# mataiyuan/ASD-SLAM

Measured on AMD Instinct MI355X. Metric: frames/sec end-to-end tracking+LocalBA, KITTI 00 mono @2000 keypoints, higher is better.
Workload: dtype f32

## Files before the change

### asd-slam_amd/csrc/asdnet.hip

```cpp
#include "ctx.h"

#include <algorithm>
#include <cmath>
#include <cstring>

typedef float f32x16 __attribute__((ext_vector_type(16)));
typedef float f32x4 __attribute__((ext_vector_type(4)));


namespace {

struct LayerSpec { int cout, cin, k, stride, pad; };
const LayerSpec kLayers[7] = {{32, 1, 3, 1, 1},   {32, 32, 3, 1, 1},   {64, 32, 3, 2, 1},  {64, 64, 3, 1, 1},
                              {128, 64, 3, 2, 1}, {128, 128, 3, 1, 1}, {128, 128, 8, 1, 0}};

template <int CIN, int COUT, int HIN, int S, int ROWS, int WM, int WN, int KC, int PP = 1, int RING = 2>
struct ConvCfg {
  static constexpr int HO = HIN / S;
  static constexpr int INROWS = (ROWS - 1) * S + 3;
  static constexpr int INCOLS = (HO - 1) * S + 3;
  static constexpr int CPAD = CIN + 4;
  static constexpr int NW = WM * WN;
  static constexpr int NTH = 64 * NW;
  static constexpr int M_PATCH = ROWS * HO;
// ... 412 lines not shown


constexpr float kActScale = 16.f;

typedef _Float16 f16x8 __attribute__((ext_vector_type(8)));
__device__ inline void split8_f16(const f32x4& v0, const f32x4& v1, float scale, u32x4& ph, u32x4& pl) {
  float x[8] = {v0[0], v0[1], v0[2], v0[3], v1[0], v1[1], v1[2], v1[3]};
  f16x8 h, l;
#pragma unroll
  for (int j = 0; j < 8; ++j) {
    const float xs = x[j] * scale;
    h[j] = (_Float16)xs;
    l[j] = (_Float16)(xs - (float)h[j]);
  }
  ph = __builtin_bit_cast(u32x4, h);
  pl = __builtin_bit_cast(u32x4, l);
}

__device__ __forceinline__ void split4_mix(float x0, float x1, float x2, float x3, float s, uint32_t (&h)[2], uint32_t (&l)[2]) {
  asm("v_fma_mixlo_f16 %0, %8, %4, 0\n\t"
      "v_fma_mixlo_f16 %1, %8, %6, 0\n\t"
      "v_fma_mixhi_f16 %0, %8, %5, 0\n\t"
      "v_fma_mixhi_f16 %1, %8, %7, 0\n\t"
      "v_fma_mixlo_f16 %2, %8, %4, -%0 op_sel_hi:[0,0,1]\n\t"
      "v_fma_mixlo_f16 %3, %8, %6, -%1 op_sel_hi:[0,0,1]\n\t"
      "v_fma_mixhi_f16 %2, %8, %5, -%0 op_sel:[0,0,1] op_sel_hi:[0,0,1]\n\t"
      "v_fma_mixhi_f16 %3, %8, %7, -%1 op_sel:[0,0,1] op_sel_hi:[0,0,1]\n\t"
      "s_nop 0"
      : "=&v"(h[0]), "=&v"(h[1]), "=&v"(l[0]), "=&v"(l[1])
      : "v"(x0), "v"(x1), "v"(x2), "v"(x3), "s"(s));
}


__global__ __launch_bounds__(256) void k_patch_stats(const uint8_t* __restrict__ patches, float* __restrict__ stats, int n) {
  __shared__ float red[8];
  const int t = threadIdx.x, lane = t & 63, wave = t >> 6, patch = blockIdx.x;
  const uchar4 v = reinterpret_cast<const uchar4*>(patches + (size_t)patch * 1024)[t];
  const float inv255 = (float)(1.0 / 255);
  float x[4] = {v.x * inv255, v.y * inv255, v.z * inv255, v.w * inv255};
#pragma unroll
  for (int k = 0; k < 4; ++k) asm volatile("" : "+v"(x[k]));
  float sum = (x[0] + x[1]) + (x[2] + x[3]);
  for (int off = 32; off >= 1; off >>= 1) sum += __shfl_xor(sum, off);
  if (lane == 0) red[wave] = sum;
  asd_syncthreads();
  const float mean = ((red[0] + red[1]) + (red[2] + red[3])) * (1.0f / 1024.0f);
  float d[4], ss = 0.f;
  for (int k = 0; k < 4; ++k) { d[k] = x[k] - mean; ss += d[k] * d[k]; }
  for (int off = 32; off >= 1; off >>= 1) ss += __shfl_xor(ss, off);
  if (lane == 0) red[4 + wave] = ss;
  asd_syncthreads();
  const float sd = sqrtf(((red[4] + red[5]) + (red[6] + red[7])) * (1.0f / 1023.0f)) + 1e-7f;
  if (t == 0) { stats[2 * (size_t)patch] = mean; stats[2 * (size_t)patch + 1] = sd; }
}

template <int CIN, int COUT, int HIN, int S, int ROWS, int WM, int WN, int PP, bool FUSE1 = false, int NP = 3, bool PAIR = false>
__device__ __forceinline__ void conv_x3_tile(const int bid, const void* __restrict__ in_, const uint8_t* __restrict__ wimg,
                                                         const float* __restrict__ bias, float* __restrict__ out,
                                                         const float* __restrict__ w1, const float* __restrict__ b1, int n,
                                                         unsigned long long* __restrict__ stamps, float in_scale, float out_scale,
                                                         const float* __restrict__ stats = nullptr) {
  using C = X3Cfg<CIN, COUT, HIN, S, ROWS, WM, WN, PP, NP>;
  constexpr int NTH = C::NTH, MT = C::MT, NCW = C::NCW;
  static_assert(!PAIR || NP == 2, "the pair format belongs to the two-piece form");
  extern __shared__ __attribute__((aligned(16))) uint8_t smem_b[];
  int t = threadIdx.x;
  asm volatile("" : "+v"(t));
  const int lane = t & 63, wave = t >> 6;
  const int wm = wave / WN, wn = wave % WN;
  constexpr int BANDS = C::HO / ROWS;
  const int patch = (bid / BANDS) * PP, band = bid % BANDS;
  const int r0 = band * ROWS;
  unsigned long long st_t0 = 0, st_t1 = 0;
  if (stamps) st_t0 = st_t1 = __builtin_amdgcn_s_memtime();
#define X3_STAMP(k) do { if (stamps && t == 0) stamps[16 * bid + (k)] = __builtin_amdgcn_s_memtime() - st_t0; } while (0)

  constexpr int SUB = 2, KG = C::KCH / 8, TW = 32 / SUB;
  const int kg = lane >> 4, lr = lane & 15;
  const uint8_t* wl = wimg + ((size_t)kg * COUT + wn * NCW + lr) * 16;
  constexpr int NB = NCW / TW;
  auto load_b = [&](int c, u32x4 (&b)[NB][NP]) {
    const uint8_t* wc = wl + (size_t)c * C::CHUNKB;
#pragma unroll
    for (int nb = 0; nb < NB; ++nb)
#pragma unroll
      for (int p = 0; p < NP; ++p) b[nb][p] = *reinterpret_cast<const u32x4*>(wc + (size_t)p * KG * COUT * 16 + nb * TW * 16);
  };
  constexpr int RB = C::NCHUNK % ASD_X3_RB == 0 ? ASD_X3_RB : 3;
  static_assert(C::NCHUNK % RB == 0, "chunk count");
  u32x4 br[RB][NB][NP];
#pragma unroll
  for (int d = 0; d < RB - 1; ++d) load_b(d, br[d]);

  if constexpr (FUSE1) {
    static_assert(!FUSE1 || (CIN == 32 && HIN == 32 && S == 1 && PP == 1 && (C::NW == 4 || C::NW == 8)), "conv1 fusion is for conv2 only");
    float* pin = reinterpret_cast<float*>(smem_b + C::ACT_BYTES);
    float* wsh = pin + (ROWS + 4) * 36;
    float* red = wsh + 320;
    const uint8_t* patches = static_cast<const uint8_t*>(in_);
    for (int i = t; i < (ROWS + 4) * 36; i += NTH) {
      const int j = i / 36, c = i % 36, y = r0 - 2 + j;
      if (!(c >= 1 && c <= 32 && y >= 0 && y < 32)) pin[i] = 0.f;
    }
    for (int i = t; i < 288; i += NTH) wsh[i] = w1[i];
    if (t < 32) wsh[288 + t] = b1[t];
    const bool ld = C::NW == 4 || wave < 4;
    const uchar4 v = ld ? reinterpret_cast<const uchar4*>(patches + (size_t)patch * 1024)[t] : make_uchar4(0, 0, 0, 0);
    const float inv255 = (float)(1.0 / 255);
    float x[4] = {v.x * inv255, v.y * inv255, v.z * inv255, v.w * inv255};
#pragma unroll
    for (int k = 0; k < 4; ++k) asm volatile("" : "+v"(x[k]));
    float d[4], sd;
    if (stats) {
      const float mean = stats[2 * (size_t)patch];
      sd = stats[2 * (size_t)patch + 1];
      for (int k = 0; k < 4; ++k) d[k] = x[k] - mean;
      X3_STAMP(9);
    } else {
      float sum = (x[0] + x[1]) + (x[2] + x[3]);
      for (int off = 32; off >= 1; off >>= 1) sum += __shfl_xor(sum, off);
      X3_STAMP(9);
      if (lane == 0 && ld) red[wave] = sum;
      asd_syncthreads();
      const float mean = ((red[0] + red[1]) + (red[2] + red[3])) * (1.0f / 1024.0f);
      float ss = 0.f;
      for (int k = 0; k < 4; ++k) { d[k] = x[k] - mean; ss += d[k] * d[k]; }
      for (int off = 32; off >= 1; off >>= 1) ss += __shfl_xor(ss, off);
      if (lane == 0 && ld) red[4 + wave] = ss;
      asd_syncthreads();
      sd = sqrtf(((red[4] + red[5]) + (red[6] + red[7])) * (1.0f / 1023.0f)) + 1e-7f;
    }
    if (ld) {
      const int idx = t * 4, y = idx >> 5, x0 = idx & 31;
      const int j = y - (r0 - 2);
      if (j >= 0 && j < ROWS + 4)
        for (int k = 0; k < 4; ++k) pin[j * 36 + x0 + k + 1] = d[k] / sd;
    }
    asd_syncthreads();
    if (stamps) st_t1 = __builtin_amdgcn_s_memtime();
    constexpr int NPIX = C::INROWS * C::INCOLS;
    const int q = t & 3;
    float wq[8][9], bq1[8];
#pragma unroll
    for (int c = 0; c < 8; ++c) {
      bq1[c] = wsh[288 + 8 * q + c];
#pragma unroll
      for (int k = 0; k < 9; ++k) wq[c][k] = wsh[(8 * q + c) * 9 + k];
    }
    for (int item = t; item < NPIX * 4; item += NTH) {
      const int pix = item >> 2;
      const int i = pix % C::INCOLS, j = pix / C::INCOLS;
      const int oy = r0 - 1 + j, ox = i - 1;
      f32x4 ra = {0.f, 0.f, 0.f, 0.f}, rb = {0.f, 0.f, 0.f, 0.f};
      if (oy >= 0 && oy < 32 && ox >= 0 && ox < 32) {
        float a[9];
#pragma unroll
        for (int ky = 0; ky < 3; ++ky)
#pragma unroll
          for (int kx = 0; kx < 3; ++kx) a[ky * 3 + kx] = pin[(j + ky) * 36 + ox + kx];
#pragma unroll
        for (int c = 0; c < 8; ++c) {
          float acc1 = bq1[c];
#pragma unroll
          for (int k = 0; k < 9; ++k) acc1 += a[k] * wq[c][k];
          const float r = acc1 > 0.f ? acc1 : 0.f;
          if (c < 4) ra[c] = r; else rb[c - 4] = r;
        }
      }
      u32x4 ph, pm, pl;
      uint8_t* dst = smem_b + pix * C::PIXB + q * C::GSTR;
      if constexpr (NP == 2) {
        split8_f16(ra, rb, in_scale, ph, pl);
        *reinterpret_cast<u32x4*>(dst) = ph;
        *reinterpret_cast<u32x4*>(dst + C::PSTR) = pl;
      } else {
        split8(ra, rb, ph, pm, pl);
        *reinterpret_cast<u32x4*>(dst) = ph;
        *reinterpret_cast<u32x4*>(dst + 16) = pm;
        *reinterpret_cast<u32x4*>(dst + 32) = pl;
      }
    }
  } else if constexpr (PAIR) {
    const uint8_t* inb = static_cast<const uint8_t*>(in_) + (size_t)patch * HIN * HIN * CIN * 4;
    constexpr int C8 = CIN / 8;
    constexpr int NPIXB = C::INROWS * C::INCOLS;
    static_assert(NTH % C8 == 0, "a thread keeps its channel group");
    constexpr int PSTEP = NTH / C8;
// ... 135 lines not shown
#pragma unroll
      for (int ma = 0; ma < NA; ++ma) {
        const int q = u * NA + ma;
        const int qn = q + PD;
        load_a(abase[qn % NA] + offs[qn / NA], ar[qn % RS]);
        const u32x4 (&ac)[NP] = ar[q % RS];
#pragma unroll
        for (int nb = 0; nb < NB; ++nb) {
          if constexpr (NP == 2) {
            mma(ac[1], bc[nb][0], acc[ma][nb]);
            mma(ac[0], bc[nb][1], acc[ma][nb]);
            mma(ac[0], bc[nb][0], acc[ma][nb]);
          } else {
            mma(ac[2], bc[nb][0], acc[ma][nb]);
            mma(ac[0], bc[nb][2], acc[ma][nb]);
            mma(ac[1], bc[nb][1], acc[ma][nb]);
            mma(ac[1], bc[nb][0], acc[ma][nb]);
            mma(ac[0], bc[nb][1], acc[ma][nb]);
            mma(ac[0], bc[nb][0], acc[ma][nb]);
          }
        }
#pragma unroll
        for (int p = 0; p < NP; ++p) {
          __builtin_amdgcn_sched_group_barrier(0x008, (NP * (NP + 1) / 2) * NB / NP, 0);
          __builtin_amdgcn_sched_group_barrier(0x100, 1, 0);
        }
      }
    }
  }

  if (stamps) {
    asm volatile("s_nop 0" ::"v"(acc[NA - 1][NB - 1][0]));
    const unsigned long long e_c = __builtin_amdgcn_s_memtime(), e_r = __builtin_amdgcn_s_memrealtime();
    if (t == 0) { stamps[16 * bid] = e_c - st_c; stamps[16 * bid + 1] = e_r - st_r; stamps[16 * bid + 2] = st_t1 - st_t0; stamps[16 * bid + 3] = st_c - st_t1; stamps[16 * bid + 6] = st_t0; }
  }
  if constexpr (PAIR) {
    uint8_t* opb = reinterpret_cast<uint8_t*>(out) + ((size_t)patch * C::HO + r0) * C::HO * COUT * 4;
    for (int nb = 0; nb < NB; ++nb) {
      const int co0 = wn * NCW + nb * TW + 4 * kg;
      const f32x4 bv = *reinterpret_cast<const f32x4*>(bias + co0);
      for (int ma = 0; ma < NA; ++ma) {
        const int m0 = wm * MT * 32 + ma * TW;
        const int pp = PP > 1 ? m0 / C::M_PATCH : 0;
        if (PP > 1 && patch + pp >= n) continue;
        const int m = tile_pixel(m0 / TW, lr);
        float v[4];
#pragma unroll
        for (int r = 0; r < 4; ++r) { const float x = acc[ma][nb][r] * out_scale + bv[r]; v[r] = x < 0.f ? 0.f : x; }
        uint32_t hh[2], ll[2];
        split4_mix(v[0], v[1], v[2], v[3], kActScale, hh, ll);
        const auto s0 = __builtin_amdgcn_permlane16_swap(hh[0], ll[0], false, false);
        const auto s1 = __builtin_amdgcn_permlane16_swap(hh[1], ll[1], false, false);
        uint8_t* o = opb + ((size_t)pp * C::HO * C::HO + (size_t)(m - pp * C::M_PATCH)) * COUT * 4 + (co0 >> 3) * 32 + (kg & 1) * 16;
        *reinterpret_cast<u32x4*>(o) = u32x4{s0[0], s1[0], s0[1], s1[1]};
      }
    }
  } else {
  float* op = out + ((size_t)patch * C::HO + r0) * C::HO * COUT;
  for (int nb = 0; nb < NB; ++nb) {
    const int co = wn * NCW + nb * TW + lr;
    const float bv = bias[co];
    for (int ma = 0; ma < NA; ++ma) {
      const int m0 = wm * MT * 32 + ma * TW;
      const int pp = PP > 1 ? m0 / C::M_PATCH : 0;
      if (PP > 1 && patch + pp >= n) continue;
      for (int r = 0; r < AR; ++r) {
        const int m = tile_pixel(m0 / TW, 4 * kg + r);
        const size_t o = (size_t)pp * C::HO * C::HO * COUT + (size_t)(m - pp * C::M_PATCH) * COUT + co;
        const float v = (NP == 2 ? acc[ma][nb][r] * out_scale : acc[ma][nb][r]) + bv;
        op[o] = NP == 2 ? (v < 0.f ? 0.f : v) : (v > 0.f ? v : 0.f);
      }
    }
  }
  }
  if (stamps && t == 0) { const unsigned long long e = __builtin_amdgcn_s_memtime(); stamps[16 * bid + 5] = e - st_t0; stamps[16 * bid + 7] = e; }
}

#ifndef ASD_L2_MINWG
#define ASD_L2_MINWG 3
#endif
template <int CIN, int COUT, int HIN, int S, int ROWS, int WM, int WN, int PP, bool FUSE1 = false, int NP = 3, bool PAIR = false>
__global__ __launch_bounds__(64 * WM * WN, (FUSE1 && NP == 2) ? ASD_L2_MINWG : 1) void k_conv_x3(const void* __restrict__ in_, const uint8_t* __restrict__ wimg,
                                                         const float* __restrict__ bias, float* __restrict__ out,
                                                         const float* __restrict__ w1, const float* __restrict__ b1, int n,
                                                         unsigned long long* __restrict__ stamps, float in_scale, float out_scale,
                                                         const float* __restrict__ stats) {
  const int bid = (S == 2 && CIN == 32) ? (int)(gridDim.x - 1 - blockIdx.x) : (int)blockIdx.x;
  conv_x3_tile<CIN, COUT, HIN, S, ROWS, WM, WN, PP, FUSE1, NP, PAIR>(bid, in_, wimg, bias, out, w1, b1, n, stamps, in_scale, out_scale, stats);
}

constexpr int FC_SK = 16;
constexpr int FC_KCH = 128;
constexpr int FC_MT = 1;
__global__ __launch_bounds__(256) void k_fc_mfma(const float* __restrict__ act, const float* __restrict__ wimg,
                                                 float* __restrict__ part, int n, int npad) {
  __shared__ __attribute__((aligned(16))) float sa[FC_MT * 32 * (FC_KCH + 4)];
  const int t = threadIdx.x, lane = t & 63, wave = t >> 6;
  const int h = lane >> 5, li = lane & 31;
  const int p0 = blockIdx.x * 32 * FC_MT, sk = blockIdx.y;
  constexpr int KPER = 8192 / FC_SK;
  f32x16 acc[FC_MT];
  for (int m = 0; m < FC_MT; ++m)
    for (int r = 0; r < 16; ++r) acc[m][r] = 0.f;
  for (int st = 0; st < KPER / FC_KCH; ++st) {
    const int k0 = sk * KPER + st * FC_KCH;
    asd_syncthreads();
    for (int idx = t; idx < FC_MT * 32 * (FC_KCH / 4); idx += 256) {
      const int c4 = idx % (FC_KCH / 4), row = idx / (FC_KCH / 4);
      int p = p0 + row;
      if (p >= n) p = n - 1;
      *reinterpret_cast<f32x4*>(sa + row * (FC_KCH + 4) + c4 * 4) =
          *reinterpret_cast<const f32x4*>(act + (size_t)p * 8192 + k0 + c4 * 4);
    }
    asd_syncthreads();
    const float* wb = wimg + ((size_t)(k0 / 8) * 2 + h) * 128 * 4 + (wave * 32 + li) * 4;
#pragma unroll 4
    for (int c8 = 0; c8 < FC_KCH / 8; ++c8) {
      const f32x4 b = *reinterpret_cast<const f32x4*>(wb + (size_t)c8 * 2 * 128 * 4);
      f32x4 a[FC_MT];
#pragma unroll
      for (int m = 0; m < FC_MT; ++m) a[m] = *reinterpret_cast<const f32x4*>(sa + (m * 32 + li) * (FC_KCH + 4) + c8 * 8 + 4 * h);
// ... 199 lines not shown
                                                float* __restrict__ desc, int n, int npad, int* __restrict__ range_flag) {
  const int lane = threadIdx.x & 63, p = blockIdx.x * 4 + (threadIdx.x >> 6);
  if (p >= n) return;
  float v0 = 0.f, v1 = 0.f;
  for (int sk = 0; sk < FC_SK; ++sk) {
    v0 += part[((size_t)sk * npad + p) * 128 + lane];
    v1 += part[((size_t)sk * npad + p) * 128 + lane + 64];
  }
  v0 += bias[lane];
  v1 += bias[lane + 64];
  float ss = v0 * v0 + v1 * v1;
  for (int off = 32; off >= 1; off >>= 1) ss += __shfl_xor(ss, off);
  const float norm = sqrtf(ss + 1e-10f);
  if (range_flag && lane == 0 && !(fabsf(ss) <= 3.0e38f)) *range_flag = 1;
  desc[(size_t)p * 128 + lane] = v0 / norm;
  desc[(size_t)p * 128 + lane + 64] = v1 / norm;
}

#define L2_CFG 32, 32, 32, 1, 4, 4, 1, 16, 1, 3
#define L3_CFG 32, 64, 32, 2, 4, 2, 2, 16
#define L4_CFG 64, 64, 16, 1, 8, 4, 1, 32, 1, 2
#define L5_CFG 64, 128, 16, 2, 4, 1, 4, 16, 1, 3
#define L6_CFG 128, 128, 8, 1, 8, 2, 2, 16, 1, 3
#ifndef ASD_L2_WMN
#define ASD_L2_WMN 4, 1
#endif
#ifndef ASD_L3_WMN
#define ASD_L3_WMN 1, 4
#endif
#ifndef ASD_L4_WMN
#define ASD_L4_WMN 2, 2
#endif
#define L2S_CFG 32, 32, 32, 1, 8, ASD_L2_WMN, 1
#ifndef ASD_L3_ROWS
#define ASD_L3_ROWS 4
#endif
#define L3S_CFG 32, 64, 32, 2, ASD_L3_ROWS, ASD_L3_WMN, 1
#define L4S_CFG 64, 64, 16, 1, 8, ASD_L4_WMN, 1
#ifndef ASD_L5_RWMN
#define ASD_L5_RWMN 8, 1, 4
#endif
#ifndef ASD_L6_WMN
#define ASD_L6_WMN 1, 4
#endif
#define L5S_CFG 64, 128, 16, 2, ASD_L5_RWMN, 1
#define L6S_CFG 128, 128, 8, 1, 8, ASD_L6_WMN, 1

template <int CIN, int COUT, int HIN, int S, int ROWS, int WM, int WN, int KC, int PP = 1, int RING = 2, bool FUSE1 = false>
hipError_t launch_conv(hipStream_t st, const void* in, const float* wimg, const float* bias, float* out, int n,
                       const float* w1 = nullptr, const float* b1 = nullptr) {
  using C = ConvCfg<CIN, COUT, HIN, S, ROWS, WM, WN, KC, PP, RING>;
  auto kern = k_conv_mfma<CIN, COUT, HIN, S, ROWS, WM, WN, KC, PP, RING, FUSE1>;
  constexpr int lds = C::LDS_BYTES + (FUSE1 ? ((ROWS + 4) * 36 + 320 + 8) * 4 : 0);
  static_assert(lds <= 160 * 1024, "band + weight ring do not fit LDS");
  static AsdPerDeviceOnce attr_set;
  int dev_ = 0;
  (void)hipGetDevice(&dev_);
  if (attr_set.need(dev_)) {
    hipError_t e = hipFuncSetAttribute(reinterpret_cast<const void*>(kern), hipFuncAttributeMaxDynamicSharedMemorySize, lds);
    if (e != hipSuccess) return e;
    attr_set.done(dev_);
  }
  hipLaunchKernelGGL(kern, dim3(((n + PP - 1) / PP) * (C::HO / ROWS)), dim3(C::NTH), lds, st, in, wimg, bias, out, w1, b1, n);
  return hipGetLastError();
}

template <int CIN, int COUT, int HIN, int S, int ROWS, int WM, int WN, int KC>
hipError_t launch_conv_p(hipStream_t st, const float* in, const float* wimg, const float* bias, float* out, int n, int num_cu) {
  using C = ConvCfg<CIN, COUT, HIN, S, ROWS, WM, WN, KC>;
  auto kern = k_conv_mfma_p<CIN, COUT, HIN, S, ROWS, WM, WN, KC>;
  constexpr int lds = (2 * C::ACT_FLOATS + 2 * C::WCHUNK) * 4;
  static_assert(lds <= 160 * 1024, "double-buffered band does not fit LDS");
  static AsdPerDeviceOnce attr_set;
  int dev_ = 0;
  (void)hipGetDevice(&dev_);
  if (attr_set.need(dev_)) {
    hipError_t e = hipFuncSetAttribute(reinterpret_cast<const void*>(kern), hipFuncAttributeMaxDynamicSharedMemorySize, lds);
    if (e != hipSuccess) return e;
    attr_set.done(dev_);
  }
  const int ntiles = n * (C::HO / ROWS);
  const int per_cu = std::max(1, std::min(4, (160 * 1024) / lds));
  const int grid = std::min(ntiles, num_cu * per_cu);
  hipLaunchKernelGGL(kern, dim3(grid), dim3(256), lds, st, in, wimg, bias, out, ntiles);
  return hipGetLastError();
}

template <int CIN, int COUT, int HIN, int S, int ROWS, int WM, int WN, int PP, bool FUSE1 = false, int NP = 3, bool PAIR = false>
hipError_t launch_conv_x3(hipStream_t st, const void* in, const void* wimg, const float* bias, float* out, int n,
                          const float* w1 = nullptr, const float* b1 = nullptr, unsigned long long* stamps = nullptr, int* grid_out = nullptr,
                          float in_scale = 1.f, float out_scale = 1.f, const float* stats = nullptr) {
  using C = X3Cfg<CIN, COUT, HIN, S, ROWS, WM, WN, PP, NP>;
  auto kern = k_conv_x3<CIN, COUT, HIN, S, ROWS, WM, WN, PP, FUSE1, NP, PAIR>;
  constexpr int lds0 = C::LDS_BYTES + (FUSE1 ? ((ROWS + 4) * 36 + 320 + 8) * 4 : 0);
  static_assert(lds0 <= 160 * 1024, "band does not fit LDS");
  const int lds = lds0;
  static AsdPerDeviceOnce attr_set;
  int dev_ = 0;
  (void)hipGetDevice(&dev_);
  if (attr_set.need(dev_)) {
    hipError_t e = hipFuncSetAttribute(reinterpret_cast<const void*>(kern), hipFuncAttributeMaxDynamicSharedMemorySize, lds);
    if (e != hipSuccess) return e;
    attr_set.done(dev_);
  }
  const int ntiles = ((n + PP - 1) / PP) * (C::HO / ROWS);
  if (grid_out) *grid_out = ntiles;
  hipLaunchKernelGGL(kern, dim3(ntiles), dim3(C::NTH), lds, st, in, static_cast<const uint8_t*>(wimg), bias, out, w1, b1, n, stamps,
                     in_scale, out_scale, stats);
  return hipGetLastError();
}

inline void split3_host(float x, uint16_t& h, uint16_t& m, uint16_t& l) {
  uint32_t u, r1u, r2u;
  memcpy(&u, &x, 4);
  const uint32_t hu = u & 0xffff0000u;
  float hf; memcpy(&hf, &hu, 4);
  const float r1 = x - hf;
  memcpy(&r1u, &r1, 4);
  const uint32_t mu = r1u & 0xffff0000u;
  float mf; memcpy(&mf, &mu, 4);
  const float r2 = r1 - mf;
  memcpy(&r2u, &r2, 4);
  h = (uint16_t)(hu >> 16); m = (uint16_t)(mu >> 16); l = (uint16_t)(r2u >> 16);
}

inline void split2_host(float xs, uint16_t& h, uint16_t& l) {
  const _Float16 hh = (_Float16)xs;
  const _Float16 ll = (_Float16)(xs - (float)hh);
  memcpy(&h, &hh, 2);
  memcpy(&l, &ll, 2);
}

inline float weight_scale_f16(const float* w, size_t count, const std::vector<float>& inv, size_t per_cout) {
  float mx = 0.f;
  for (size_t i = 0; i < count; ++i) mx = std::max(mx, std::fabs(w[i] * inv[i / per_cout]));
  if (!(mx > 0.f) || !std::isfinite(mx)) return 1.f;
  int e;
  (void)std::frexp(mx, &e);
  return std::ldexp(1.f, 14 - e);
}

// ... 8 lines not shown
        uint16_t p[3];
        if (np == 3) split3_host(v, p[0], p[1], p[2]);
        else split2_host(v * wscale, p[0], p[1]);
        const int c16 = ci / kch, hh = (ci % kch) / 8, j = ci % 8;
        for (int q = 0; q < np; ++q)
          img[(((((size_t)tap * nc16 + c16) * np + q) * kg + hh) * L.cout + co) * 8 + j] = p[q];
      }
}

void build_wimg(const LayerSpec& L, const float* w, const std::vector<float>& inv, std::vector<float>& img) {
  img.assign((size_t)9 * L.cin * L.cout, 0.f);
  for (int tap = 0; tap < 9; ++tap)
    for (int ci = 0; ci < L.cin; ++ci)
      for (int co = 0; co < L.cout; ++co) {
        const int c8 = ci / 8, hh = (ci % 8) / 4, jj = ci % 4;
        const size_t dst = ((((size_t)tap * (L.cin / 8) + c8) * 2 + hh) * L.cout + co) * 4 + jj;
        img[dst] = w[((size_t)co * L.cin + ci) * 9 + tap] * inv[co];
      }
}

}

int asdnet_alloc(asd_ctx* ctx) {
  const size_t np = (size_t)ctx->cfg.max_patches;
  const size_t npad = (np + 31) / 32 * 32;
  ASD_HIP_CHECK(ctx, hipMalloc(&ctx->d_act[0], np * 32768 * sizeof(float)));
  ASD_HIP_CHECK(ctx, hipMalloc(&ctx->d_act[1], np * 32768 * sizeof(float)));
  ASD_HIP_CHECK(ctx, hipMalloc(&ctx->d_part, (size_t)FC_SK * npad * 128 * sizeof(float)));
  ASD_HIP_CHECK(ctx, hipMalloc(&ctx->d_patches, np * 1024));
  ASD_HIP_CHECK(ctx, hipMalloc(&ctx->d_desc, np * 128 * sizeof(float)));
  ASD_HIP_CHECK(ctx, hipHostMalloc(reinterpret_cast<void**>(&ctx->h_range), 64));
  *ctx->h_range = 0;
  if (const char* e = getenv("ASD_ASDNET_PAIR")) ctx->net_pair = atoi(e) != 0;
  return ASD_OK;
}

void asdnet_free(asd_ctx* ctx) {
  for (int i = 0; i < 2; ++i) if (ctx->d_act[i]) (void)hipFree(ctx->d_act[i]);
  if (ctx->d_part) (void)hipFree(ctx->d_part);
  if (ctx->d_patches) (void)hipFree(ctx->d_patches);
  if (ctx->d_desc) (void)hipFree(ctx->d_desc);
  if (ctx->h_range) (void)hipHostFree(ctx->h_range);
  if (ctx->d_w1) (void)hipFree(ctx->d_w1);
  for (int i = 0; i < 7; ++i) {
    if (ctx->d_bias[i]) (void)hipFree(ctx->d_bias[i]);
    if (ctx->d_wimg[i]) (void)hipFree(ctx->d_wimg[i]);
    if (ctx->d_wx3[i]) (void)hipFree(ctx->d_wx3[i]);
    if (ctx->d_wx2[i]) (void)hipFree(ctx->d_wx2[i]);
  }
}

static int asdnet_calibrate(asd_ctx* ctx, const float* const conv_w[7], const float* const bn_mean[7], const float* const bn_var[7], float eps);

int asdnet_load_weights(asd_ctx* ctx, const float* const conv_w[7], const float* const bn_mean[7],
                        const float* const bn_var[7], float eps) {
  for (int l = 0; l < 7; ++l) {
    const LayerSpec& L = kLayers[l];
    std::vector<float> inv(L.cout), bias(L.cout);
    for (int c = 0; c < L.cout; ++c) {
      inv[c] = 1.0f / std::sqrt(bn_var[l][c] + eps);
      bias[c] = -bn_mean[l][c] * inv[c];
    }
    if (!ctx->d_bias[l]) ASD_HIP_CHECK(ctx, hipMalloc(&ctx->d_bias[l], L.cout * sizeof(float)));
    ASD_HIP_CHECK(ctx, hipMemcpy(ctx->d_bias[l], bias.data(), L.cout * sizeof(float), hipMemcpyHostToDevice));
    std::vector<float> img;
    if (l == 0) {
// ... 54 lines not shown
      if (!ctx->d_wx2[l]) ASD_HIP_CHECK(ctx, hipMalloc(&ctx->d_wx2[l], x3.size() * sizeof(uint16_t)));
      ASD_HIP_CHECK(ctx, hipMemcpy(ctx->d_wx2[l], x3.data(), x3.size() * sizeof(uint16_t), hipMemcpyHostToDevice));
    }
  }
  ctx->weights_loaded = true;
  return asdnet_calibrate(ctx, conv_w, bn_mean, bn_var, eps);
}

int asdnet_profile_collect_set(asd_ctx* ctx, int set);

static int asdnet_forward_one(asd_ctx* ctx, const uint8_t* d_patches, int n, float* d_desc, hipStream_t st, int* range_flag);
int asdnet_forward_device(asd_ctx* ctx, const uint8_t* d_patches, int n, float* d_desc, hipStream_t st, int* range_flag) {
  if (!ctx->weights_loaded) { ctx->set_error("asd_load_weights has not been called"); return ASD_ERR_NO_WEIGHTS; }
  if (n < 0 || n > ctx->cfg.max_patches) { ctx->set_error("n=%d exceeds max_patches=%d", n, ctx->cfg.max_patches); return ASD_ERR_CAPACITY; }
  if (n == 0) return ASD_OK;
  if (!st) st = ctx->stream;
  std::lock_guard<std::mutex> prof_lock(ctx->prof_mutex);
  return asdnet_forward_one(ctx, d_patches, n, d_desc, st, range_flag);
}
static int asdnet_forward_one(asd_ctx* ctx, const uint8_t* d_patches, int n, float* d_desc, hipStream_t st, int* range_flag) {
  float *a0 = ctx->d_act[0], *a1 = ctx->d_act[1];
  const int npad = (n + 31) / 32 * 32;
  const bool prof = ctx->prof_on;
  const int pset = ctx->prof_cur;
  if (prof && ctx->prof_pending[pset]) { int rc = asdnet_profile_collect_set(ctx, pset); if (rc != ASD_OK) return rc; }
#define PROF_MARK(i) do { if (prof) ASD_HIP_CHECK(ctx, hipEventRecord(ctx->prof_ev[pset][i], st)); } while (0)
  PROF_MARK(0);
  PROF_MARK(1);
#define CALIB(l, buf, elems) do { if (ctx->d_calib) { hipLaunchKernelGGL(k_absmax, dim3(256), dim3(256), 0, st, buf, (size_t)n * (elems), ctx->d_calib + (l)); ASD_HIP_CHECK(ctx, hipGetLastError()); } } while (0)
  ctx->d_act6 = a1;
  if (ctx->net_split) {
    const bool p2 = ctx->net_pieces == 2;
    const bool pair = p2 && ctx->net_pair && !ctx->d_calib;
    const float* x3_stats = nullptr;
#define X3_LAUNCH(CFG, FUSE, l, src, dst, w1p, b1p)                                                                                       \
  (pair ? launch_conv_x3<CFG, FUSE, 2, true>(st, src, ctx->d_wx2[l], ctx->d_bias[l], dst, n, w1p, b1p, nullptr, nullptr, kActScale,          \
                                     1.f / (kActScale * ctx->wx2_scale[l]), x3_stats)                                                               \
   : p2 ? launch_conv_x3<CFG, FUSE, 2>(st, src, ctx->d_wx2[l], ctx->d_bias[l], dst, n, w1p, b1p, nullptr, nullptr, kActScale,               \
                                     1.f / (kActScale * ctx->wx2_scale[l]), x3_stats)                                                               \
      : launch_conv_x3<CFG, FUSE, 3>(st, src, ctx->d_wx3[l], ctx->d_bias[l], dst, n, w1p, b1p, nullptr, nullptr, 1.f, 1.f,                \
                                     x3_stats))
    hipLaunchKernelGGL(k_patch_stats, dim3(n), dim3(256), 0, st, d_patches, ctx->d_part, n);
    ASD_HIP_CHECK(ctx, hipGetLastError());
    x3_stats = ctx->d_part;
    ASD_HIP_CHECK(ctx, (X3_LAUNCH(L2S_CFG, true, 1, d_patches, a1, ctx->d_w1, ctx->d_bias[0])));
    x3_stats = nullptr;
    CALIB(1, a1, 32 * 32 * 32);
    PROF_MARK(2);
    ASD_HIP_CHECK(ctx, (X3_LAUNCH(L3S_CFG, false, 2, a1, a0, nullptr, nullptr)));
    CALIB(2, a0, 16 * 16 * 64);
    PROF_MARK(3);
    ASD_HIP_CHECK(ctx, (X3_LAUNCH(L4S_CFG, false, 3, a0, a1, nullptr, nullptr)));
    CALIB(3, a1, 16 * 16 * 64);
    PROF_MARK(4);
    ASD_HIP_CHECK(ctx, (X3_LAUNCH(L5S_CFG, false, 4, a1, a0, nullptr, nullptr)));
    CALIB(4, a0, 8 * 8 * 128);
    PROF_MARK(5);
    ASD_HIP_CHECK(ctx, (X3_LAUNCH(L6S_CFG, false, 5, a0, a1, nullptr, nullptr)));
#undef X3_LAUNCH
    CALIB(5, a1, 8 * 8 * 128);
    PROF_MARK(6);
    if (pair)
      hipLaunchKernelGGL(k_fc_x2, dim3((npad + FCS_MP - 1) / FCS_MP, FC_SK), dim3(256), 0, st, reinterpret_cast<const uint8_t*>(a1),
                         static_cast<const uint8_t*>(ctx->d_wx2[6]), ctx->d_part, n, npad, 1.f / (kActScale * ctx->wx2_scale[6]));
    else
      hipLaunchKernelGGL(k_fc_x3, dim3((npad + FCS_MP - 1) / FCS_MP, FC_SK), dim3(256), 0, st, a1, static_cast<const uint8_t*>(ctx->d_wx3[6]), ctx->d_part, n, npad);
  } else {
    ASD_HIP_CHECK(ctx, (launch_conv<L2_CFG, true>(st, d_patches, ctx->d_wimg[1], ctx->d_bias[1], a1, n, ctx->d_w1, ctx->d_bias[0])));
    CALIB(1, a1, 32 * 32 * 32);
    PROF_MARK(2);
    ASD_HIP_CHECK(ctx, (launch_conv_p<L3_CFG>(st, a1, ctx->d_wimg[2], ctx->d_bias[2], a0, n, ctx->num_cu)));
    CALIB(2, a0, 16 * 16 * 64);
    PROF_MARK(3);
    ASD_HIP_CHECK(ctx, (launch_conv<L4_CFG>(st, a0, ctx->d_wimg[3], ctx->d_bias[3], a1, n)));
    CALIB(3, a1, 16 * 16 * 64);
    PROF_MARK(4);
    ASD_HIP_CHECK(ctx, (launch_conv<L5_CFG>(st, a1, ctx->d_wimg[4], ctx->d_bias[4], a0, n)));
    CALIB(4, a0, 8 * 8 * 128);
    PROF_MARK(5);
// ... 111 lines not shown
    ctx->prof_patches[l] += ctx->prof_pending_n[set];
  }
  ctx->prof_pending[set] = false;
  return ASD_OK;
}

int asdnet_profile_collect(asd_ctx* ctx) {
  std::lock_guard<std::mutex> prof_lock(ctx->prof_mutex);
  for (int set = 0; set < 2; ++set) {
    const int rc = asdnet_profile_collect_set(ctx, set);
    if (rc != ASD_OK) return rc;
  }
  return ASD_OK;
}

extern "C" int asd_debug_act6(asd_ctx* ctx, int n, float* out) {
  if (n < 0 || n > ctx->cfg.max_patches) return ASD_ERR_CAPACITY;
  ASD_HIP_CHECK(ctx, hipStreamSynchronize(ctx->stream));
  const bool pair = ctx->net_pieces == 2 && ctx->net_split && ctx->net_pair;
  const float* src = ctx->d_act6 ? ctx->d_act6 : ctx->d_act[1];
  if (!pair) { ASD_HIP_CHECK(ctx, hipMemcpy(out, src, (size_t)n * 8192 * 4, hipMemcpyDeviceToHost)); return ASD_OK; }
  std::vector<uint16_t> raw((size_t)n * 8192 * 2);
  ASD_HIP_CHECK(ctx, hipMemcpy(raw.data(), src, raw.size() * 2, hipMemcpyDeviceToHost));
  for (size_t e = 0; e < (size_t)n * 8192; ++e) {
    const size_t g = e / 8, j = e % 8;
    _Float16 h, l;
    memcpy(&h, &raw[g * 16 + j], 2);
    memcpy(&l, &raw[g * 16 + 8 + j], 2);
    out[e] = ((float)h + (float)l) / kActScale;
  }
  return ASD_OK;
}

extern "C" int asd_debug_x3_clock(asd_ctx* ctx, int layer, int n, int reps, double* loop_cycles, double* ghz) {
  hipStream_t st = ctx->stream;
  float *a0 = ctx->d_act[0], *a1 = ctx->d_act[1];
  unsigned long long* stamps = reinterpret_cast<unsigned long long*>(ctx->d_part);
  int grid = 0;
  for (int r = 0; r < reps; ++r) {
    unsigned long long* sp = r + 1 == reps ? stamps : nullptr;
    hipError_t e = hipErrorInvalidValue;
    const bool p2 = ctx->net_pieces == 2;
    const bool pair = p2 && ctx->net_pair;
#define X3_CLK(CFG, FUSE, l, src, dst, w1p, b1p)                                                                                          \
  (pair ? launch_conv_x3<CFG, FUSE, 2, true>(st, src, ctx->d_wx2[l], ctx->d_bias[l], dst, n, w1p, b1p, sp, &grid, kActScale,                  \
                                     1.f / (kActScale * ctx->wx2_scale[l]))                                                                \
   : p2 ? launch_conv_x3<CFG, FUSE, 2>(st, src, ctx->d_wx2[l], ctx->d_bias[l], dst, n, w1p, b1p, sp, &grid, kActScale,                       \
                                     1.f / (kActScale * ctx->wx2_scale[l]))                                                                \
      : launch_conv_x3<CFG, FUSE, 3>(st, src, ctx->d_wx3[l], ctx->d_bias[l], dst, n, w1p, b1p, sp, &grid))
    if (layer == 2) e = X3_CLK(L2S_CFG, true, 1, ctx->d_patches, a1, ctx->d_w1, ctx->d_bias[0]);
    else if (layer == 3) e = X3_CLK(L3S_CFG, false, 2, a1, a0, nullptr, nullptr);
    else if (layer == 4) e = X3_CLK(L4S_CFG, false, 3, a0, a1, nullptr, nullptr);
    else if (layer == 5) e = X3_CLK(L5S_CFG, false, 4, a1, a0, nullptr, nullptr);
    else if (layer == 6) e = X3_CLK(L6S_CFG, false, 5, a0, a1, nullptr, nullptr);
#undef X3_CLK
    ASD_HIP_CHECK(ctx, e);
  }
  ASD_HIP_CHECK(ctx, hipStreamSynchronize(st));
  if ((size_t)grid * 128 > (size_t)FC_SK * ((ctx->cfg.max_patches + 31) / 32 * 32) * 128 * sizeof(float)) return ASD_ERR_CAPACITY;
  std::vector<unsigned long long> hs((size_t)grid * 16);
  ASD_HIP_CHECK(ctx, hipMemcpy(hs.data(), stamps, hs.size() * 8, hipMemcpyDeviceToHost));
  std::vector<double> cyc(grid), rate(grid);
  for (int i = 0; i < grid; ++i) { cyc[i] = (double)hs[16 * i]; rate[i] = hs[16 * i + 1] ? (double)hs[16 * i] / (double)hs[16 * i + 1] : 0.0; }
  std::nth_element(cyc.begin(), cyc.begin() + grid / 2, cyc.end());
  std::nth_element(rate.begin(), rate.begin() + grid / 2, rate.end());
  *loop_cycles = cyc[grid / 2];
  *ghz = rate[grid / 2] * 0.1;
  if (getenv("ASD_X3_PHASES")) {
    auto med = [&](int k) { std::vector<double> v(grid); for (int i = 0; i < grid; ++i) v[i] = (double)hs[16 * i + k]; std::nth_element(v.begin(), v.begin() + grid / 2, v.end()); return v[grid / 2]; };
    fprintf(stderr, "  layer %d: %d workgroups; prologue %.0f, staging %.0f, MFMA loop %.0f, whole life %.0f cycles (medians)\n", layer, grid, med(2), med(3),
            med(0), med(5));
    if (layer == 2) fprintf(stderr, "     since entry: patch arrived %.0f, staging loop done %.0f, barrier passed %.0f\n", med(9), med(12), med(13));
  }
  return ASD_OK;
}
```

### asd-slam_amd/csrc/ctx.h

```cpp
#pragma once
#include <hip/hip_runtime.h>

#include <atomic>
#include <cstdarg>
#include <cstdio>
#include <cstdlib>
#include <cstring>
#include <functional>
#include <mutex>
#include <string>
#include <vector>

#include "../../include/asd_slam.h"

#define ASD_HIP_CHECK(ctx, expr)                                                          \
  do {                                                                                    \
    hipError_t _e = (expr);                                                               \
    if (_e != hipSuccess) {                                                               \
      (ctx)->set_error("%s failed: %s (%s:%d)", #expr, hipGetErrorString(_e), __FILE__, __LINE__); \
      return ASD_ERR_HIP;                                                                 \
    }                                                                                     \
  } while (0)

struct AsdPerDeviceOnce {
// ... 193 lines not shown
  asd_config cfg{};
  hipStream_t stream = nullptr;
  hipStream_t stream_x = nullptr;
  hipStream_t stream_prep = nullptr;
  hipEvent_t ev_prep = nullptr;
  bool prep_on = false;
  struct AsyncExtract* ax = nullptr;
  int num_cu = 256;
  std::string err;

  float scale[ASD_MAX_LEVELS], inv_scale[ASD_MAX_LEVELS], sigma2[ASD_MAX_LEVELS], inv_sigma2[ASD_MAX_LEVELS];
  int features_per_level[ASD_MAX_LEVELS];
  float level_thr[ASD_MAX_LEVELS];
  int umax[16];

  bool weights_loaded = false;
  float* d_w1 = nullptr;
  float* d_bias[7] = {};
  float* d_wimg[7] = {};
  void* d_wx3[7] = {};
  bool match_replay_host = false;
  bool ba_struct_host = false;
  void* d_wx2[7] = {};
  float wx2_scale[7] = {1, 1, 1, 1, 1, 1, 1};
  int net_pieces_req = 2;
  int net_pieces = 2;
  int net_split = 0x3f;
  float* d_act[2] = {};
  float* d_part = nullptr;
  int* h_range = nullptr;
  std::string calib_note;
  unsigned* d_calib = nullptr;
  bool net_pair = true;
  float* d_act6 = nullptr;
  uint8_t* d_patches = nullptr;
  int patches_n = 0;
  float* d_desc = nullptr;
  bool keep_pyramid = false;
  const uint8_t* d_pyr_view = nullptr;
  AsdDevBuf stereo_scratch;
  float* d_desc_last = nullptr;
  hipEvent_t ev_adopt = nullptr;
  bool adopt_pending = false;

  struct FrontendState* fe = nullptr;
  UndistortMap* und = nullptr;
  int last_n = 0;

  AsdFrameSlot frames[ASD_MAX_FRAMES];

  void* matcher = nullptr;

  void* ba = nullptr;

  AsdDevBuf scratch;
  AsdXfer up, down;
  bool track_async_armed = false, track_has_pending = false;
  hipEvent_t ev_chain = nullptr;
  std::function<int()> track_pending;

  void* mapping = nullptr;

  void* bow = nullptr;

  void* sim3 = nullptr;

// ... 91 lines not shown
```

Before: 1326.

## Process four conv2 bands per workgroup, computing patch stats once and carrying halo rows

The fused conv1+conv2 kernel now processes several row bands of the same patch in one workgroup (four by default on the pair path). Patch mean and standard deviation are computed once per workgroup, which removes the separate patch-stats kernel launch and its global round trip. Between bands, the two overlapping conv1 output rows already held in LDS are moved forward instead of recomputed, and padding columns are zeroed once. The cost is fewer workgroups, so less parallelism and a longer serial chain per workgroup, plus extra registers for the carried halo.

After: 1324. Within noise of the previous version (-0.2%).

```diff
diff --git a/asd-slam_amd/csrc/asdnet.hip b/asd-slam_amd/csrc/asdnet.hip
--- a/asd-slam_amd/csrc/asdnet.hip
+++ b/asd-slam_amd/csrc/asdnet.hip
@@ -468,48 +468,74 @@
 }
 
 
-__global__ __launch_bounds__(256) void k_patch_stats(const uint8_t* __restrict__ patches, float* __restrict__ stats, int n) {
-  __shared__ float red[8];
-  const int t = threadIdx.x, lane = t & 63, wave = t >> 6, patch = blockIdx.x;
-  const uchar4 v = reinterpret_cast<const uchar4*>(patches + (size_t)patch * 1024)[t];
-  const float inv255 = (float)(1.0 / 255);
-  float x[4] = {v.x * inv255, v.y * inv255, v.z * inv255, v.w * inv255};
-#pragma unroll
-  for (int k = 0; k < 4; ++k) asm volatile("" : "+v"(x[k]));
-  float sum = (x[0] + x[1]) + (x[2] + x[3]);
-  for (int off = 32; off >= 1; off >>= 1) sum += __shfl_xor(sum, off);
-  if (lane == 0) red[wave] = sum;
-  asd_syncthreads();
-  const float mean = ((red[0] + red[1]) + (red[2] + red[3])) * (1.0f / 1024.0f);
-  float d[4], ss = 0.f;
-  for (int k = 0; k < 4; ++k) { d[k] = x[k] - mean; ss += d[k] * d[k]; }
-  for (int off = 32; off >= 1; off >>= 1) ss += __shfl_xor(ss, off);
-  if (lane == 0) red[4 + wave] = ss;
-  asd_syncthreads();
-  const float sd = sqrtf(((red[4] + red[5]) + (red[6] + red[7])) * (1.0f / 1023.0f)) + 1e-7f;
-  if (t == 0) { stats[2 * (size_t)patch] = mean; stats[2 * (size_t)patch + 1] = sd; }
-}
-
-template <int CIN, int COUT, int HIN, int S, int ROWS, int WM, int WN, int PP, bool FUSE1 = false, int NP = 3, bool PAIR = false>
+template <int CIN, int COUT, int HIN, int S, int ROWS, int WM, int WN, int PP, bool FUSE1 = false, int NP = 3, bool PAIR = false, int BPW = 1>
 __device__ __forceinline__ void conv_x3_tile(const int bid, const void* __restrict__ in_, const uint8_t* __restrict__ wimg,
                                                          const float* __restrict__ bias, float* __restrict__ out,
                                                          const float* __restrict__ w1, const float* __restrict__ b1, int n,
-                                                         unsigned long long* __restrict__ stamps, float in_scale, float out_scale,
-                                                         const float* __restrict__ stats = nullptr) {
+                                                         unsigned long long* __restrict__ stamps, float in_scale, float out_scale) {
   using C = X3Cfg<CIN, COUT, HIN, S, ROWS, WM, WN, PP, NP>;
   constexpr int NTH = C::NTH, MT = C::MT, NCW = C::NCW;
   static_assert(!PAIR || NP == 2, "the pair format belongs to the two-piece form");
   extern __shared__ __attribute__((aligned(16))) uint8_t smem_b[];
+  constexpr int BANDS = C::HO / ROWS;
+  static_assert(BPW == 1 || (FUSE1 && BANDS % BPW == 0), "several bands per workgroup: conv2 only, whole patches");
+  const int tile0 = bid * BPW;
+  const int patch = (tile0 / BANDS) * PP;
   int t = threadIdx.x;
   asm volatile("" : "+v"(t));
+  unsigned long long st_t0 = 0, st_t1 = 0;
+  if (stamps) st_t0 = st_t1 = __builtin_amdgcn_s_memtime();
+  int tile = tile0;
+#define X3_STAMP(k) do { if (stamps && t == 0) stamps[16 * tile + (k)] = __builtin_amdgcn_s_memtime() - st_t0; } while (0)
+
+  float xn[4] = {0.f, 0.f, 0.f, 0.f};
+  if constexpr (FUSE1) {
+    static_assert(!FUSE1 || (CIN == 32 && HIN == 32 && S == 1 && PP == 1 && (C::NW == 4 || C::NW == 8)), "conv1 fusion is for conv2 only");
+    float* pin = reinterpret_cast<float*>(smem_b + C::ACT_BYTES);
+    float* wsh = pin + (ROWS + 4) * 36;
+    float* red = wsh + 320;
+    const uint8_t* patches = static_cast<const uint8_t*>(in_);
+    const int lane = t & 63, wave = t >> 6;
+    const bool ld = C::NW == 4 || wave < 4;
+    const uchar4 v = ld ? reinterpret_cast<const uchar4*>(patches + (size_t)patch * 1024)[t] : make_uchar4(0, 0, 0, 0);
+    for (int i = t; i < (ROWS + 4) * 4; i += NTH) pin[(i >> 2) * 36 + ((i & 3) ? 32 + (i & 3) : 0)] = 0.f;
+    constexpr int PSLOTS = (C::PIXB - 16) / 16;
+    for (int i = t; i < C::INROWS * 2 * PSLOTS; i += NTH) {
+      const int p = i / PSLOTS, s = i % PSLOTS;
+      *reinterpret_cast<u32x4*>(smem_b + ((p >> 1) * C::INCOLS + (p & 1) * (C::INCOLS - 1)) * C::PIXB + s * 16) = u32x4{0, 0, 0, 0};
+    }
+    for (int i = t; i < 288; i += NTH) wsh[i] = w1[i];
+    if (t < 32) wsh[288 + t] = b1[t];
+    const float inv255 = (float)(1.0 / 255);
+    float x[4] = {v.x * inv255, v.y * inv255, v.z * inv255, v.w * inv255};
+#pragma unroll
+    for (int k = 0; k < 4; ++k) asm volatile("" : "+v"(x[k]));
+    float sum = (x[0] + x[1]) + (x[2] + x[3]);
+    for (int off = 32; off >= 1; off >>= 1) sum += __shfl_xor(sum, off);
+    X3_STAMP(9);
+    if (lane == 0 && ld) red[wave] = sum;
+    asd_syncthreads();
+    const float mean = ((red[0] + red[1]) + (red[2] + red[3])) * (1.0f / 1024.0f);
+    float d[4], ss = 0.f;
+    for (int k = 0; k < 4; ++k) { d[k] = x[k] - mean; ss += d[k] * d[k]; }
+    for (int off = 32; off >= 1; off >>= 1) ss += __shfl_xor(ss, off);
+    if (lane == 0 && ld) red[4 + wave] = ss;
+    asd_syncthreads();
+    const float sd = sqrtf(((red[4] + red[5]) + (red[6] + red[7])) * (1.0f / 1023.0f)) + 1e-7f;
+    for (int k = 0; k < 4; ++k) xn[k] = d[k] / sd;
+  }
+
+  for (int bi = 0; bi < BPW; ++bi) {
+  if constexpr (BPW > 1) {
+    asm volatile("" : "+v"(t));
+    tile = tile0 + bi;
+    if (stamps && bi) st_t0 = st_t1 = __builtin_amdgcn_s_memtime();
+  }
   const int lane = t & 63, wave = t >> 6;
   const int wm = wave / WN, wn = wave % WN;
-  constexpr int BANDS = C::HO / ROWS;
-  const int patch = (bid / BANDS) * PP, band = bid % BANDS;
+  const int band = tile % BANDS;
   const int r0 = band * ROWS;
-  unsigned long long st_t0 = 0, st_t1 = 0;
-  if (stamps) st_t0 = st_t1 = __builtin_amdgcn_s_memtime();
-#define X3_STAMP(k) do { if (stamps && t == 0) stamps[16 * bid + (k)] = __builtin_amdgcn_s_memtime() - st_t0; } while (0)
+  if (stamps && t == 0) stamps[16 * tile + 8] = bi == 0;
 
   constexpr int SUB = 2, KG = C::KCH / 8, TW = 32 / SUB;
   const int kg = lane >> 4, lr = lane & 15;
@@ -529,52 +555,36 @@
   for (int d = 0; d < RB - 1; ++d) load_b(d, br[d]);
 
   if constexpr (FUSE1) {
-    static_assert(!FUSE1 || (CIN == 32 && HIN == 32 && S == 1 && PP == 1 && (C::NW == 4 || C::NW == 8)), "conv1 fusion is for conv2 only");
     float* pin = reinterpret_cast<float*>(smem_b + C::ACT_BYTES);
     float* wsh = pin + (ROWS + 4) * 36;
-    float* red = wsh + 320;
-    const uint8_t* patches = static_cast<const uint8_t*>(in_);
-    for (int i = t; i < (ROWS + 4) * 36; i += NTH) {
-      const int j = i / 36, c = i % 36, y = r0 - 2 + j;
-      if (!(c >= 1 && c <= 32 && y >= 0 && y < 32)) pin[i] = 0.f;
-    }
-    for (int i = t; i < 288; i += NTH) wsh[i] = w1[i];
-    if (t < 32) wsh[288 + t] = b1[t];
-    const bool ld = C::NW == 4 || wave < 4;
-    const uchar4 v = ld ? reinterpret_cast<const uchar4*>(patches + (size_t)patch * 1024)[t] : make_uchar4(0, 0, 0, 0);
-    const float inv255 = (float)(1.0 / 255);
-    float x[4] = {v.x * inv255, v.y * inv255, v.z * inv255, v.w * inv255};
-#pragma unroll
-    for (int k = 0; k < 4; ++k) asm volatile("" : "+v"(x[k]));
-    float d[4], sd;
-    if (stats) {
-      const float mean = stats[2 * (size_t)patch];
-      sd = stats[2 * (size_t)patch + 1];
-      for (int k = 0; k < 4; ++k) d[k] = x[k] - mean;
-      X3_STAMP(9);
-    } else {
-      float sum = (x[0] + x[1]) + (x[2] + x[3]);
-      for (int off = 32; off >= 1; off >>= 1) sum += __shfl_xor(sum, off);
-      X3_STAMP(9);
-      if (lane == 0 && ld) red[wave] = sum;
-      asd_syncthreads();
-      const float mean = ((red[0] + red[1]) + (red[2] + red[3])) * (1.0f / 1024.0f);
-      float ss = 0.f;
-      for (int k = 0; k < 4; ++k) { d[k] = x[k] - mean; ss += d[k] * d[k]; }
-      for (int off = 32; off >= 1; off >>= 1) ss += __shfl_xor(ss, off);
-      if (lane == 0 && ld) red[4 + wave] = ss;
-      asd_syncthreads();
-      sd = sqrtf(((red[4] + red[5]) + (red[6] + red[7])) * (1.0f / 1023.0f)) + 1e-7f;
-    }
-    if (ld) {
+    if (C::NW == 4 || wave < 4) {
       const int idx = t * 4, y = idx >> 5, x0 = idx & 31;
       const int j = y - (r0 - 2);
       if (j >= 0 && j < ROWS + 4)
-        for (int k = 0; k < 4; ++k) pin[j * 36 + x0 + k + 1] = d[k] / sd;
+        for (int k = 0; k < 4; ++k) pin[j * 36 + x0 + k + 1] = xn[k];
+    }
+    for (int i = t; i < (ROWS + 4) * 32; i += NTH) {
+      const int j = i >> 5, y = r0 - 2 + j;
+      if (y < 0 || y >= 32) pin[j * 36 + 1 + (i & 31)] = 0.f;
+    }
+    constexpr int HPIX = 2 * 32 * ((C::PIXB - 16) / 16);
+    constexpr int HN = (HPIX + NTH - 1) / NTH;
+    u32x4 halo[HN];
+    const bool carry = bi > 0;
+    auto halo_off = [&](int e) { const int p = e / ((C::PIXB - 16) / 16), s = e % ((C::PIXB - 16) / 16); return (((p >> 5) * C::INCOLS + 1 + (p & 31)) * C::PIXB + s * 16); };
+    if (carry) {
+#pragma unroll
+      for (int u = 0; u < HN; ++u)
+        if (t + u * NTH < HPIX) halo[u] = *reinterpret_cast<const u32x4*>(smem_b + ROWS * C::INCOLS * C::PIXB + halo_off(t + u * NTH));
     }
     asd_syncthreads();
     if (stamps) st_t1 = __builtin_amdgcn_s_memtime();
-    constexpr int NPIX = C::INROWS * C::INCOLS;
+    if (carry) {
+#pragma unroll
+      for (int u = 0; u < HN; ++u)
+        if (t + u * NTH < HPIX) *reinterpret_cast<u32x4*>(smem_b + halo_off(t + u * NTH)) = halo[u];
+    }
+    const int jlo = carry ? 2 : 0;
     const int q = t & 3;
     float wq[8][9], bq1[8];
 #pragma unroll
@@ -583,12 +593,12 @@
 #pragma unroll
       for (int k = 0; k < 9; ++k) wq[c][k] = wsh[(8 * q + c) * 9 + k];
     }
-    for (int item = t; item < NPIX * 4; item += NTH) {
-      const int pix = item >> 2;
-      const int i = pix % C::INCOLS, j = pix / C::INCOLS;
-      const int oy = r0 - 1 + j, ox = i - 1;
+    for (int item = t; item < (C::INROWS - jlo) * 32 * 4; item += NTH) {
+      const int j = jlo + (item >> 7), ox = (item >> 2) & 31;
+      const int pix = j * C::INCOLS + ox + 1;
+      const int oy = r0 - 1 + j;
       f32x4 ra = {0.f, 0.f, 0.f, 0.f}, rb = {0.f, 0.f, 0.f, 0.f};
-      if (oy >= 0 && oy < 32 && ox >= 0 && ox < 32) {
+      if (oy >= 0 && oy < 32) {
         float a[9];
 #pragma unroll
         for (int ky = 0; ky < 3; ++ky)
@@ -790,7 +800,7 @@
   if (stamps) {
     asm volatile("s_nop 0" ::"v"(acc[NA - 1][NB - 1][0]));
     const unsigned long long e_c = __builtin_amdgcn_s_memtime(), e_r = __builtin_amdgcn_s_memrealtime();
-    if (t == 0) { stamps[16 * bid] = e_c - st_c; stamps[16 * bid + 1] = e_r - st_r; stamps[16 * bid + 2] = st_t1 - st_t0; stamps[16 * bid + 3] = st_c - st_t1; stamps[16 * bid + 6] = st_t0; }
+    if (t == 0) { stamps[16 * tile] = e_c - st_c; stamps[16 * tile + 1] = e_r - st_r; stamps[16 * tile + 2] = st_t1 - st_t0; stamps[16 * tile + 3] = st_c - st_t1; stamps[16 * tile + 6] = st_t0; }
   }
   if constexpr (PAIR) {
     uint8_t* opb = reinterpret_cast<uint8_t*>(out) + ((size_t)patch * C::HO + r0) * C::HO * COUT * 4;
@@ -831,20 +841,20 @@
     }
   }
   }
-  if (stamps && t == 0) { const unsigned long long e = __builtin_amdgcn_s_memtime(); stamps[16 * bid + 5] = e - st_t0; stamps[16 * bid + 7] = e; }
+  if (stamps && t == 0) { const unsigned long long e = __builtin_amdgcn_s_memtime(); stamps[16 * tile + 5] = e - st_t0; stamps[16 * tile + 7] = e; }
+  }
 }
 
 #ifndef ASD_L2_MINWG
 #define ASD_L2_MINWG 3
 #endif
-template <int CIN, int COUT, int HIN, int S, int ROWS, int WM, int WN, int PP, bool FUSE1 = false, int NP = 3, bool PAIR = false>
+template <int CIN, int COUT, int HIN, int S, int ROWS, int WM, int WN, int PP, bool FUSE1 = false, int NP = 3, bool PAIR = false, int BPW = 1>
 __global__ __launch_bounds__(64 * WM * WN, (FUSE1 && NP == 2) ? ASD_L2_MINWG : 1) void k_conv_x3(const void* __restrict__ in_, const uint8_t* __restrict__ wimg,
                                                          const float* __restrict__ bias, float* __restrict__ out,
                                                          const float* __restrict__ w1, const float* __restrict__ b1, int n,
-                                                         unsigned long long* __restrict__ stamps, float in_scale, float out_scale,
-                                                         const float* __restrict__ stats) {
+                                                         unsigned long long* __restrict__ stamps, float in_scale, float out_scale) {
   const int bid = (S == 2 && CIN == 32) ? (int)(gridDim.x - 1 - blockIdx.x) : (int)blockIdx.x;
-  conv_x3_tile<CIN, COUT, HIN, S, ROWS, WM, WN, PP, FUSE1, NP, PAIR>(bid, in_, wimg, bias, out, w1, b1, n, stamps, in_scale, out_scale, stats);
+  conv_x3_tile<CIN, COUT, HIN, S, ROWS, WM, WN, PP, FUSE1, NP, PAIR, BPW>(bid, in_, wimg, bias, out, w1, b1, n, stamps, in_scale, out_scale);
 }
 
 constexpr int FC_SK = 16;
@@ -1110,6 +1120,7 @@
 #define ASD_L4_WMN 2, 2
 #endif
 #define L2S_CFG 32, 32, 32, 1, 8, ASD_L2_WMN, 1
+constexpr int L2S_BPW = 4;
 #ifndef ASD_L3_ROWS
 #define ASD_L3_ROWS 4
 #endif
@@ -1164,12 +1175,12 @@
   return hipGetLastError();
 }
 
-template <int CIN, int COUT, int HIN, int S, int ROWS, int WM, int WN, int PP, bool FUSE1 = false, int NP = 3, bool PAIR = false>
+template <int CIN, int COUT, int HIN, int S, int ROWS, int WM, int WN, int PP, bool FUSE1 = false, int NP = 3, bool PAIR = false, int BPW = 1>
 hipError_t launch_conv_x3(hipStream_t st, const void* in, const void* wimg, const float* bias, float* out, int n,
                           const float* w1 = nullptr, const float* b1 = nullptr, unsigned long long* stamps = nullptr, int* grid_out = nullptr,
-                          float in_scale = 1.f, float out_scale = 1.f, const float* stats = nullptr) {
+                          float in_scale = 1.f, float out_scale = 1.f) {
   using C = X3Cfg<CIN, COUT, HIN, S, ROWS, WM, WN, PP, NP>;
-  auto kern = k_conv_x3<CIN, COUT, HIN, S, ROWS, WM, WN, PP, FUSE1, NP, PAIR>;
+  auto kern = k_conv_x3<CIN, COUT, HIN, S, ROWS, WM, WN, PP, FUSE1, NP, PAIR, BPW>;
   constexpr int lds0 = C::LDS_BYTES + (FUSE1 ? ((ROWS + 4) * 36 + 320 + 8) * 4 : 0);
   static_assert(lds0 <= 160 * 1024, "band does not fit LDS");
   const int lds = lds0;
@@ -1183,8 +1194,8 @@
   }
   const int ntiles = ((n + PP - 1) / PP) * (C::HO / ROWS);
   if (grid_out) *grid_out = ntiles;
-  hipLaunchKernelGGL(kern, dim3(ntiles), dim3(C::NTH), lds, st, in, static_cast<const uint8_t*>(wimg), bias, out, w1, b1, n, stamps,
-                     in_scale, out_scale, stats);
+  hipLaunchKernelGGL(kern, dim3(ntiles / BPW), dim3(C::NTH), lds, st, in, static_cast<const uint8_t*>(wimg), bias, out, w1, b1, n, stamps,
+                     in_scale, out_scale);
   return hipGetLastError();
 }
 
@@ -1259,6 +1270,7 @@
   ASD_HIP_CHECK(ctx, hipHostMalloc(reinterpret_cast<void**>(&ctx->h_range), 64));
   *ctx->h_range = 0;
   if (const char* e = getenv("ASD_ASDNET_PAIR")) ctx->net_pair = atoi(e) != 0;
+  if (const char* e = getenv("ASD_ASDNET_CONV2")) ctx->net_conv2_bands = strcmp(e, "bands") == 0;
   return ASD_OK;
 }
 
@@ -1379,19 +1391,17 @@
   if (ctx->net_split) {
     const bool p2 = ctx->net_pieces == 2;
     const bool pair = p2 && ctx->net_pair && !ctx->d_calib;
-    const float* x3_stats = nullptr;
 #define X3_LAUNCH(CFG, FUSE, l, src, dst, w1p, b1p)                                                                                       \
   (pair ? launch_conv_x3<CFG, FUSE, 2, true>(st, src, ctx->d_wx2[l], ctx->d_bias[l], dst, n, w1p, b1p, nullptr, nullptr, kActScale,          \
-                                     1.f / (kActScale * ctx->wx2_scale[l]), x3_stats)                                                               \
+                                     1.f / (kActScale * ctx->wx2_scale[l]))                                                                \
    : p2 ? launch_conv_x3<CFG, FUSE, 2>(st, src, ctx->d_wx2[l], ctx->d_bias[l], dst, n, w1p, b1p, nullptr, nullptr, kActScale,               \
-                                     1.f / (kActScale * ctx->wx2_scale[l]), x3_stats)                                                               \
-      : launch_conv_x3<CFG, FUSE, 3>(st, src, ctx->d_wx3[l], ctx->d_bias[l], dst, n, w1p, b1p, nullptr, nullptr, 1.f, 1.f,                \
-                                     x3_stats))
-    hipLaunchKernelGGL(k_patch_stats, dim3(n), dim3(256), 0, st, d_patches, ctx->d_part, n);
-    ASD_HIP_CHECK(ctx, hipGetLastError());
-    x3_stats = ctx->d_part;
-    ASD_HIP_CHECK(ctx, (X3_LAUNCH(L2S_CFG, true, 1, d_patches, a1, ctx->d_w1, ctx->d_bias[0])));
-    x3_stats = nullptr;
+                                     1.f / (kActScale * ctx->wx2_scale[l]))                                                                \
+      : launch_conv_x3<CFG, FUSE, 3>(st, src, ctx->d_wx3[l], ctx->d_bias[l], dst, n, w1p, b1p, nullptr, nullptr, 1.f, 1.f))
+    if (pair && !ctx->net_conv2_bands)
+      ASD_HIP_CHECK(ctx, (launch_conv_x3<L2S_CFG, true, 2, true, L2S_BPW>(st, d_patches, ctx->d_wx2[1], ctx->d_bias[1], a1, n, ctx->d_w1, ctx->d_bias[0], nullptr,
+                                                                         nullptr, kActScale, 1.f / (kActScale * ctx->wx2_scale[1]))));
+    else
+      ASD_HIP_CHECK(ctx, (X3_LAUNCH(L2S_CFG, true, 1, d_patches, a1, ctx->d_w1, ctx->d_bias[0])));
     CALIB(1, a1, 32 * 32 * 32);
     PROF_MARK(2);
     ASD_HIP_CHECK(ctx, (X3_LAUNCH(L3S_CFG, false, 2, a1, a0, nullptr, nullptr)));
@@ -1569,6 +1579,10 @@
   return ASD_OK;
 }
 
+extern "C" int asd_debug_conv2_bands_per_wg(asd_ctx* ctx) {
+  return ctx->net_split && ctx->net_pieces == 2 && ctx->net_pair && !ctx->net_conv2_bands ? L2S_BPW : 1;
+}
+
 extern "C" int asd_debug_x3_clock(asd_ctx* ctx, int layer, int n, int reps, double* loop_cycles, double* ghz) {
   hipStream_t st = ctx->stream;
   float *a0 = ctx->d_act[0], *a1 = ctx->d_act[1];
@@ -1585,7 +1599,10 @@
    : p2 ? launch_conv_x3<CFG, FUSE, 2>(st, src, ctx->d_wx2[l], ctx->d_bias[l], dst, n, w1p, b1p, sp, &grid, kActScale,                       \
                                      1.f / (kActScale * ctx->wx2_scale[l]))                                                                \
       : launch_conv_x3<CFG, FUSE, 3>(st, src, ctx->d_wx3[l], ctx->d_bias[l], dst, n, w1p, b1p, sp, &grid))
-    if (layer == 2) e = X3_CLK(L2S_CFG, true, 1, ctx->d_patches, a1, ctx->d_w1, ctx->d_bias[0]);
+    if (layer == 2 && pair && !ctx->net_conv2_bands)
+      e = launch_conv_x3<L2S_CFG, true, 2, true, L2S_BPW>(st, ctx->d_patches, ctx->d_wx2[1], ctx->d_bias[1], a1, n, ctx->d_w1, ctx->d_bias[0], sp, &grid, kActScale,
+                                                          1.f / (kActScale * ctx->wx2_scale[1]));
+    else if (layer == 2) e = X3_CLK(L2S_CFG, true, 1, ctx->d_patches, a1, ctx->d_w1, ctx->d_bias[0]);
     else if (layer == 3) e = X3_CLK(L3S_CFG, false, 2, a1, a0, nullptr, nullptr);
     else if (layer == 4) e = X3_CLK(L4S_CFG, false, 3, a0, a1, nullptr, nullptr);
     else if (layer == 5) e = X3_CLK(L5S_CFG, false, 4, a1, a0, nullptr, nullptr);
@@ -1607,7 +1624,22 @@
     auto med = [&](int k) { std::vector<double> v(grid); for (int i = 0; i < grid; ++i) v[i] = (double)hs[16 * i + k]; std::nth_element(v.begin(), v.begin() + grid / 2, v.end()); return v[grid / 2]; };
     fprintf(stderr, "  layer %d: %d workgroups; prologue %.0f, staging %.0f, MFMA loop %.0f, whole life %.0f cycles (medians)\n", layer, grid, med(2), med(3),
             med(0), med(5));
-    if (layer == 2) fprintf(stderr, "     since entry: patch arrived %.0f, staging loop done %.0f, barrier passed %.0f\n", med(9), med(12), med(13));
+    if (layer == 2) {
+      auto medf = [&](int k, bool first) {
+        std::vector<double> v;
+        for (int i = 0; i < grid; ++i) if ((hs[16 * i + 8] != 0) == first) v.push_back((double)hs[16 * i + k]);
+        if (v.empty()) return 0.0;
+        std::nth_element(v.begin(), v.begin() + v.size() / 2, v.end());
+        return v[v.size() / 2];
+      };
+      int nfirst = 0;
+      for (int i = 0; i < grid; ++i) nfirst += hs[16 * i + 8] != 0;
+      fprintf(stderr, "     %d tiles with the workgroup's prologue: patch arrived %.0f, prologue %.0f, staging %.0f, staging loop done %.0f, barrier passed %.0f, whole %.0f\n",
+              nfirst, medf(9, true), medf(2, true), medf(3, true), medf(12, true), medf(13, true), medf(5, true));
+      if (nfirst < grid)
+        fprintf(stderr, "     %d tiles behind them:                   prologue %.0f, staging %.0f, staging loop done %.0f, barrier passed %.0f, whole %.0f\n", grid - nfirst,
+                medf(2, false), medf(3, false), medf(12, false), medf(13, false), medf(5, false));
+    }
   }
   return ASD_OK;
 }
diff --git a/asd-slam_amd/csrc/ctx.h b/asd-slam_amd/csrc/ctx.h
--- a/asd-slam_amd/csrc/ctx.h
+++ b/asd-slam_amd/csrc/ctx.h
@@ -249,6 +249,7 @@
   std::string calib_note;
   unsigned* d_calib = nullptr;
   bool net_pair = true;
+  bool net_conv2_bands = false;
   float* d_act6 = nullptr;
   uint8_t* d_patches = nullptr;
   int patches_n = 0;
```
